# thalesfm/differentiable-renderer

Measured on AMD Instinct MI355X. Metric: Mray/s (fwd+bwd), Cornell 512x512 @64spp depth 8, higher is better.
Workload: dtype f32; 1 GPU; config 3: Cornell 512x512, 64 spp, depth 8, fwd + radiative backprop w.r.t. the albedos; scene 'cornell' (cornell box of render.cpp:26-59) 512x512, 64 spp per GPU, depth 8 (-b 8 -p 1), fwd + radiative-backprop gradients of 4 parameters; program=builtin, parallelism=1 GPU, gpu_max_hw_queues=4 (set by this script before the HIP runtime started)

## Files before the change

### differentiable-renderer_amd/csrc/drt_ctx.h

```cpp
#pragma once

namespace {

struct DevBuf {
    void* p = nullptr;
    size_t cap = 0;
};

struct TimedLaunch {
    int kernel;
    hipEvent_t e0, e1;
};

struct RenderJob {
    drt_camera_desc cam;
    drt_render_params rp;
    const float* adjoint_rgb = nullptr;
    float* out_rgb = nullptr;
    double* out_param_grad = nullptr;
    float* out_gimg = nullptr;
    drt_hip_stats* stats = nullptr;
    int gimg_param = -1;
    bool backward = false, dev_out = false, timing = false, want_segments = false, sync = true;
    bool zero_copy = false;
// ... 4 lines not shown
    uint32_t n_local_pixels = 0;
    size_t n_count_words = 0;
    float* d_out = nullptr;
    float* d_gimg = nullptr;
    size_t off_grad = 0, off_img = 0, off_gimg = 0, off_adj = 0, img_bytes = 0, grad_bytes = 0;
    drt_hip_stats st;
    std::chrono::steady_clock::time_point t0;
};

}

struct drt_hip_ctx {
    int device = 0;
    int n_cu = 256;
    uint64_t device_mem = (uint64_t)288 << 30;
    int mesh_blocks_per_cu = 4;
    hipStream_t stream = nullptr;
    std::string err;

    bool has_scene = false;
    bool has_specular = false;
    bool emissive_bxdf = false;
    int max_colour_param = -1;
    bool prog_ok = false;
    bool prog_sorted = false;
    unsigned long long prog_sig[4] = {0, 0, 0, 0};
    std::string arch = "gfx950";
    int jit_mode = 1;
    uint64_t scene_work = 0;
    std::map<std::string, hipFunction_t> jit_fn;
    std::vector<hipModule_t> jit_modules;
    std::string user_header;
    std::string jit_error;
    double jit_ms = 0;
    int n_params = 0, n_shapes = 0;
    int n_user_params = 0;
    int n_grad_slots = 0;
    std::vector<uint8_t> requires_grad;
    std::vector<drt_material_desc> materials;
    DevScene<float>* d_scene_f = nullptr;
    DevScene<double>* d_scene_d = nullptr;
    float* d_params_f = nullptr;
    double* d_params_d = nullptr;
    bool has_mesh = false;
    DevBvh<float> bvh_f{};
    DevBvh<double> bvh_d{};
// ... 114 lines not shown
```

### differentiable-renderer_amd/csrc/drt_path.h

```cpp
#pragma once

#include "drt_kernels.h"

#define DRT_DRAW_TABLE (3 * DRT_MAX_DEPTH + 8)

struct PathArgs {
    int32_t W, H, spp;
    int32_t shard, n_shards, band;
    uint32_t Pb, p0, Sb, s0, spr, n_ranges, n_groups;
    int32_t min_bounces, depth_cap, cap_is_roulette, cap_draws;
    uint32_t rr_threshold, seed, rng_stream;
    uint32_t regen_min;
    uint32_t shade_min, descend_min;
    int32_t gimg_param;
    uint32_t gen_rows, gen_clog2;
    uint32_t hist_lds, hist_stride;
    uint32_t gimg_row, pad_gen;
    unsigned long long hist_ovf;
    double p_rr, inv_p_rr;
    double eye[3], fwd[3], right[3], up[3];
    double tan_half, aspect, inv_W, inv_H;
    float p_rr_f, inv_p_rr_f;
    float eye_f[3], fwd_f[3], right_f[3], up_f[3], cs_step_f, ct_step_f;
};
// ... 70 lines not shown
            dst[i] = src[i];
    }
    {
        const int* src = reinterpret_cast<const int*>(sc->materials);
        int* dst = reinterpret_cast<int*>(lds.sc.materials);
        for (int i = threadIdx.x; i < nm * (int)(sizeof(DevMaterial<R>) / sizeof(int)); i += blockDim.x)
            dst[i] = src[i];
    }
    for (int i = threadIdx.x; i < ne; i += blockDim.x)
        lds.sc.emitter_param[i] = sc->emitter_param[i];
    for (int i = threadIdx.x; i < ns; i += blockDim.x)
        lds.sc.flat[i] = sc->flat[i];
#ifdef DRT_USER_SHAPES
    for (int i = threadIdx.x; i < ns * 4; i += blockDim.x)
        lds.user_q[i >> 2][i & 3] = sc->user_q[i >> 2][i & 3];
#endif
    const int np = sc->n_params < DRT_PATH_LDS_PARAMS ? sc->n_params : DRT_PATH_LDS_PARAMS;
    for (int i = threadIdx.x; i < np * 3; i += blockDim.x)
        lds.params[i] = params[i];
    __syncthreads();
}


template <typename R>
struct TangentLds {
    R colnz[DRT_FAST_PARAMS][4];
    R invc[DRT_FAST_PARAMS][4];
    uint32_t inc[DRT_FAST_PARAMS][4];
};

template <typename R, typename SL>
__device__ inline void stage_tangents(TangentLds<R>& tl, const SL& lds)
{
    if (threadIdx.x < DRT_FAST_PARAMS) {
        const int p = threadIdx.x;
        const bool in = p < lds.sc.n_params;
        uint32_t zinc = 0, zbits = 0;
#pragma unroll
        for (int ch = 0; ch < 3; ++ch) {
            const R c = in ? lds.params[p * 3 + ch] : R(1);
            const bool zero = abs_r(c) < R(1e-18);
            tl.colnz[p][ch] = zero ? R(1) : c;
            tl.invc[p][ch] = zero ? R(0) : R(1) / c;
            zinc |= zero ? 1u << (8 * ch) : 0u;
            zbits |= zero ? 1u << ch : 0u;
        }
        tl.colnz[p][3] = R(0);
        tl.invc[p][3] = R(0);
        tl.inc[p][0] = p < 4 ? 1u << (8 * p) : 0u;
        tl.inc[p][1] = p >= 4 ? 1u << (8 * (p - 4)) : 0u;
        tl.inc[p][2] = zinc;
        tl.inc[p][3] = zbits;
    }
    __syncthreads();
}

template <typename R, int NP, int NC>
struct Tangents {
    uint32_t cnt[NC > 4 ? 2 : 1];
    uint32_t zc;
    R* acc;
    __device__ inline V3<R> acc_get(int p) const { return mk<R>(acc[(p * 3) * DRT_BLOCK], acc[(p * 3 + 1) * DRT_BLOCK], acc[(p * 3 + 2) * DRT_BLOCK]); }
    __device__ inline void acc_set(int p, V3<R> v) { acc[(p * 3) * DRT_BLOCK] = v.x; acc[(p * 3 + 1) * DRT_BLOCK] = v.y; acc[(p * 3 + 2) * DRT_BLOCK] = v.z; }
    __device__ inline void new_path() { cnt[0] = 0; if (NC > 4) cnt[NC > 4 ? 1 : 0] = 0; zc = 0; }
};

#define DRT_NP_ANY (-1)
#ifndef DRT_LOCKSTEP_MIN_BLOCKS
#define DRT_LOCKSTEP_MIN_BLOCKS 7
#endif
#ifndef DRT_LOCKSTEP_GEN_MIN_BLOCKS
#define DRT_LOCKSTEP_GEN_MIN_BLOCKS 6
#endif
#ifndef DRT_LOCKSTEP_SPEC_MIN_BLOCKS
#define DRT_LOCKSTEP_SPEC_MIN_BLOCKS 6
// ... 143 lines not shown
    tg.gsum = mk<R>(R(0), R(0), R(0));
    tg.gimg_row = a.gimg_row;
    tg.hist_lds = a.hist_lds;
    tg.hist_stride = a.hist_stride;
    tg.clog2 = a.gen_clog2;
    tg.table = &gb.table[threadIdx.x / DRT_WAVE][threadIdx.x & ((1u << a.gen_clog2) - 1u)];
    tg.acc = nullptr;
    tg.new_path();
}
template <typename R>
__device__ inline void gen_finish(const GenBlock<R>& gb, const PathArgs& a, double* __restrict__ gpart)
{
    __syncthreads();
    const uint32_t copies = 1u << a.gen_clog2;
    for (uint32_t r = threadIdx.x; r < a.gen_rows; r += DRT_BLOCK) {
        double v = 0;
        for (int ww = 0; ww < DRT_BLOCK / DRT_WAVE; ++ww)
            for (uint32_t c = 0; c < copies; ++c)
                v += (double)gb.table[ww][(r << a.gen_clog2) + c];
        gpart[(size_t)blockIdx.x * a.gen_rows + r] = v;
    }
}

template <typename R, int NP, int NC, bool LOSS = false, typename SL = PathSceneLds<R>>
__device__ inline void add_emission(const SL& lds, const TangentLds<R>& tl, const R* __restrict__ params, uint32_t eid, R inv_pk,
                                    V3<R> T, V3<R> g, V3<R>& L, Tangents<R, NP, NC>& tg)
{
    const V3<R> E = load_param<R, (NP != 0)>(lds, params, (int)eid) * inv_pk;
    V3<R> Tr = T;
    if (NC > 0 || NP == DRT_NP_ANY)
        Tr = mk<R>((tg.zc & 0xFFu) ? R(0) : T.x, (tg.zc & 0xFF00u) ? R(0) : T.y, (tg.zc & 0xFF0000u) ? R(0) : T.z);
    L = L + Tr * E;
    if constexpr (NP == DRT_NP_ANY) {
        if (LOSS)
            g = mk<R>(R(2) * (L.x - g.x), R(2) * (L.y - g.y), R(2) * (L.z - g.z));
        const V3<R> gE = g * E;
        const uint32_t ebits = pid_unpack(tg.gl->invc[eid < DRT_PATH_LDS_PARAMS ? eid : 0][3]);
        if ((ebits & 0xFFFFu) != DRT_SLOT_NONE && eid < DRT_PATH_LDS_PARAMS)
            tg.add(ebits & 0xFFFFu, g * Tr * inv_pk);
        const V3<R> TgE = Tr * gE;
        const V3<R> U = mk<R>((tg.zc & 0xFFu) == 0x1u ? T.x * gE.x : R(0), (tg.zc & 0xFF00u) == 0x100u ? T.y * gE.y : R(0),
                              (tg.zc & 0xFF0000u) == 0x10000u ? T.z * gE.z : R(0));
        const uint32_t nw = tg.nv >> 2;
        for (uint32_t w = 0; wave_any(w < nw); ++w)
            tg.add_word(w < nw ? tg.load_word(w) : 0xFFFFFFFFu, TgE, U);
        tg.add_word(tg.cur, TgE, U);
    } else
    if constexpr (NP > 0) {
        if (NC > 0)
            asm volatile("" ::: "memory");
        if (LOSS)
            g = mk<R>(R(2) * (L.x - g.x), R(2) * (L.y - g.y), R(2) * (L.z - g.z));
        const V3<R> gE = g * E, gT = g * Tr * inv_pk;
#pragma unroll
        for (int p = 0; p < NP; ++p) {
            const bool own = eid == (uint32_t)p;
            const V3<R> ap = tg.acc_get(p);
            const V3<R> a0 = mk<R>(ap.x + (own ? gT.x : R(0)), ap.y + (own ? gT.y : R(0)), ap.z + (own ? gT.z : R(0)));
            if (p < NC) {
                const uint32_t n = (tg.cnt[p >> 2] >> (8 * (p & 3))) & 0xFFu;
                const R nf = (R)(int)n;
                V3<R> dT = mk<R>(Tr.x * (nf * tl.invc[p][0]), Tr.y * (nf * tl.invc[p][1]), Tr.z * (nf * tl.invc[p][2]));
                const uint32_t zb = __builtin_amdgcn_readfirstlane(tl.inc[p][3]);
                if (zb) {
                    const bool one = n == 1u;
                    if (zb & 1u) dT.x = (one && (tg.zc & 0xFFu) == 0x1u) ? T.x : R(0);
                    if (zb & 2u) dT.y = (one && (tg.zc & 0xFF00u) == 0x100u) ? T.y : R(0);
                    if (zb & 4u) dT.z = (one && (tg.zc & 0xFF0000u) == 0x10000u) ? T.z : R(0);
                }
                tg.acc_set(p, mk<R>(fma_r(dT.x, gE.x, a0.x), fma_r(dT.y, gE.y, a0.y), fma_r(dT.z, gE.z, a0.z)));
            } else
                tg.acc_set(p, a0);
        }
    }
}

template <typename R>
struct CameraLane {
    R cs0, ct0;
};

template <typename R>
struct PathVertex {
    V3<R> P, nrm, d;
    uint32_t ids;
    int material;
    bool hit, scattered;
};

template <typename R, bool SPEC, int NP, int NC, typename SG>
__device__ inline void path_bounce(const PathArgs& a, const PathSceneLds<R>& lds, const TangentLds<R>& tl, const DevScene<R>* __restrict__ sc,
                                   const R* __restrict__ params, const ProgRecs<SG::n, R>& recs, uint32_t key,
                                   R pk, R inv_pk, uint32_t n_theta, bool next_rr, bool next_cap, bool live, V3<R> g,
                                   typename Q4<R>::T& ra, typename Q2<R>::T& rb, V3<R>& T, V3<R>& L, Tangents<R, NP, NC>& tg,
                                   bool& alive, bool& capped, bool& on_light, uint32_t& light, PathVertex<R>* vo = nullptr,
                                   bool last = false, const float* __restrict__ seed_px = nullptr, const uint32_t* ih = nullptr)
{
    auto draw = [&](uint32_t n) { return ih ? drt_rng_combine(ih[n], key) : rng_draw(a.rng_stream, key, n); };
    const HitRec<R> h = path_closest_hit<SG>(sc, recs, ra, rb);
    const bool hit = live && h.prim >= 0;
    const int prim = h.prim >= 0 ? h.prim : 0;
    const V3<R> o = mk<R>(ra.x, ra.y, ra.z);
    const V3<R> d = mk<R>(ra.w, rb.x, rb.y);
    const V3<R> P = o + d * h.t;
    const DevShape<R>& sh = lds.sc.shapes[prim];
    const uint32_t ids = (uint32_t)sh.pad;
    const uint32_t cid = ids & 0xFFFFu, eid = ids >> 16;
    const bool has_bxdf = cid != DRT_ID_NONE, emits = hit && eid != DRT_ID_NONE;
    on_light = emits && !has_bxdf;
    light = eid;
    if (last && !vo) {
        if (wave_any(emits && has_bxdf)) {
            if (emits && has_bxdf) {
// ... 23 lines not shown
    if (vo) {
        vo->P = P; vo->nrm = nrm; vo->d = d;
        vo->ids = ids;
        vo->material = sh.material;
        vo->hit = hit;
        vo->scattered = hit && has_bxdf;
    }
    if (wave_any(emits && has_bxdf)) {
        if (emits && has_bxdf) {
            if (NP != 0 && seed_px)
                g = mk<R>((R)seed_px[0], (R)seed_px[1], (R)seed_px[2]);
            add_emission<R, NP, NC>(lds, tl, params, eid, inv_pk, T, g, L, tg);
        }
    }
    const DevMaterial<R>& m = lds.sc.materials[has_bxdf ? sh.material : 0];
    V3<R> wo;
    R q, bs;
    sample_bxdf<R, SPEC>(m, nrm, d, draw(n_theta), draw(n_theta + 1), wo, q, bs);
    const R c = dot(nrm, wo);
    const R mk_ = div_r(bs * c, q * pk);
    const bool rr_kills = next_rr && draw(n_theta + 2) < a.rr_threshold;
    alive = hit && has_bxdf && !next_cap && !rr_kills;
    capped = hit && has_bxdf && next_cap && !a.cap_is_roulette && !rr_kills;
    const int cidx = has_bxdf ? (int)cid : 0;
    V3<R> col;
    if constexpr (NP == DRT_NP_ANY) {
        const R* rec = tg.gl->colnz[cidx < DRT_PATH_LDS_PARAMS ? cidx : 0];
        col = mk<R>(rec[0], rec[1], rec[2]);
        tg.zc += alive ? pid_unpack(rec[3]) : 0u;
        if (ih)
            tg.template push<false>(alive, cid);
        else
            tg.template push<true>(live, alive ? cid : 0xFFu);
    } else
        col = NC > 0 ? mk<R>(tl.colnz[cidx][0], tl.colnz[cidx][1], tl.colnz[cidx][2]) : load_param<R, (NP > 0)>(lds, params, cidx);
    const V3<R> cmv = col * mk_;
    const V3<R> cm = mk<R>(alive ? cmv.x : R(1), alive ? cmv.y : R(1), alive ? cmv.z : R(1));
    if constexpr (NC > 0 && NP != DRT_NP_ANY) {
        tg.cnt[0] += alive ? tl.inc[cidx][0] : 0u;
        if (NC > 4)
            tg.cnt[NC > 4 ? 1 : 0] += alive ? tl.inc[cidx][1] : 0u;
        tg.zc += alive ? tl.inc[cidx][2] : 0u;
    }
    T = T * cm;
    const V3<R> no = P + wo * R(1e-3);
    ra.x = no.x; ra.y = no.y; ra.z = no.z; ra.w = wo.x;
    rb.x = wo.y; rb.y = wo.z;
}

#ifndef DRT_CAMERA_ARGS_F32
#define DRT_CAMERA_ARGS_F32 1
#endif
template <typename R, bool ARGS_F32 = (DRT_CAMERA_ARGS_F32 != 0)>
__device__ inline uint32_t path_camera(const PathArgs& a, const CameraLane<R>& cl, uint32_t gpix, uint32_t px, uint32_t py, uint32_t sl,
                                       typename Q4<R>::T& ra, typename Q2<R>::T& rb)
{
    const uint64_t path = (uint64_t)gpix * (uint64_t)a.spp + (uint64_t)(a.s0 + sl);
    const uint32_t key = (uint32_t)path;
    if (sizeof(R) == 4) {
        const float cs_step = ARGS_F32 ? a.cs_step_f : (float)(2. * a.aspect * a.tan_half * a.inv_W);
// ... 36 lines not shown
    return path_camera<R, false>(a, cl, gpix, px, py, sl, ra, rb);
}

#ifndef DRT_LEAN_MAX_SHAPES
#ifdef DRT_USER_SHAPES
#define DRT_LEAN_MAX_SHAPES (-1)
#else
#define DRT_LEAN_MAX_SHAPES 10
#endif
#endif
template <size_t RB, bool SPEC, int NP, int NSG, bool REGEN>
constexpr int path_min_blocks()
{
    if (RB == 4 && NP <= 4) {
        if (!REGEN)
            return SPEC ? ((NP == DRT_NP_ANY || NSG > DRT_LEAN_MAX_SHAPES) ? 5 : DRT_LOCKSTEP_SPEC_MIN_BLOCKS)
                        : (NP == DRT_NP_ANY ? DRT_LOCKSTEP_GEN_MIN_BLOCKS : (NSG <= DRT_LEAN_MAX_SHAPES ? DRT_LOCKSTEP_MIN_BLOCKS : DRT_LOCKSTEP_GEN_MIN_BLOCKS));
        return (NP == DRT_NP_ANY && NSG == 0) ? 4
                                              : (SPEC ? 5 : DRT_REGEN_MIN_BLOCKS);
    }
    return (RB == 8 && NP <= 4 && !REGEN && !SPEC) ? DRT_F64_MIN_BLOCKS : 1;
}

template <typename R, bool SPEC, int NP, int NC, typename SG, bool REGEN = false, bool LOSS = false>
__global__ void __launch_bounds__(DRT_BLOCK, (path_min_blocks<sizeof(R), SPEC, NP, SG::n, REGEN>()))
k_path(PathArgs a, const DevScene<R>* __restrict__ sc, const R* __restrict__ params, const float* __restrict__ adjoint,
       double* __restrict__ gpart, double* __restrict__ fpart, uint32_t* __restrict__ counts,
       unsigned long long* __restrict__ total, double* __restrict__ gimg_part)
{
    if (total && blockIdx.x == 0 && threadIdx.x < 8)
        total[threadIdx.x] = 0;
    typedef typename Q4<R>::T R4;
    typedef typename Q2<R>::T R2;
    __shared__ PathSceneLds<R> lds;
    __shared__ double s_red[REGEN ? 1 : DRT_BLOCK / DRT_WAVE][DRT_FAST_PARAMS * 3];
    __shared__ TangentLds<R> s_tl;
    constexpr bool GEN = NP == DRT_NP_ANY;
    __shared__ typename PickT<GEN, GenBlock<R>, NoLds>::T s_gen;
    extern __shared__ uint32_t s_hist[];
    if constexpr (GEN)
        gen_zero(s_gen);
    stage_path_scene(lds, sc, params);
    const TangentLds<R>& tl = s_tl;
    if (NC > 0 && !GEN)
        stage_tangents(s_tl, lds);

    const uint32_t lane = threadIdx.x & (DRT_WAVE - 1);
    const uint32_t w = grid_wave();
    const uint32_t range = w / a.n_groups, group = w - range * a.n_groups;
    const uint32_t lp = group * DRT_WAVE + lane;
    const bool have = range < a.n_ranges && lp < a.Pb;
    const uint32_t s_begin = range * a.spr;
    const uint32_t s_end = s_begin + a.spr < a.Sb ? s_begin + a.spr : a.Sb;

    Tangents<R, NP, NC> tg;
    __shared__ R s_acc[NP > 0 ? NP * 3 : 1][DRT_BLOCK];
// ... 41 lines not shown
    if (range < a.n_ranges && !REGEN) {
    for (uint32_t sl = s_begin; sl < s_end; ++sl) {
        R4 ra;
        R2 rb;
        const uint32_t key = path_camera<R, ARGS_F32>(a, cl, gpix, px, py, sl, ra, rb);
        bool live = have && a.depth_cap > 0 && !(a.min_bounces <= 0 && rng_draw(a.rng_stream, key, 2) < a.rr_threshold);
        V3<R> T = mk<R>(R(1), R(1), R(1)), L = mk<R>(R(0), R(0), R(0));
        uint32_t end_ids = DRT_ID_NONE;
        R end_inv_pk = R(1);
        if (NC > 0 || GEN)
            tg.new_path();
        for (int kk = 0; kk < a.depth_cap; ++kk) {
            const uint32_t n_live = (uint32_t)__popcll(wave_ballot(live));
            if (n_live == 0)
                break;
            n_seg += n_live;
            const R pk = kk >= a.min_bounces ? pk_rr : R(1);
            const R inv_pk = kk >= a.min_bounces ? inv_p_rr : R(1);
            const uint32_t n_theta = draw_offset(kk, 0, a.min_bounces) + camera_draw_base(a.min_bounces);
            const bool next_rr = (kk + 1) >= a.min_bounces;
            const bool next_cap = (kk + 1) >= a.depth_cap;
            bool alive, capped, on_light;
            uint32_t light;
            path_bounce<R, SPEC, NP, NC, SG>(a, lds, tl, sc, params, recs, key, pk, inv_pk, n_theta, next_rr, next_cap, live, g,
                                                    ra, rb, T, L, tg, alive, capped, on_light, light, nullptr, next_cap);
            end_ids = on_light ? light : end_ids;
            end_inv_pk = on_light ? inv_pk : end_inv_pk;
            if (next_cap && !a.cap_is_roulette)
                n_capped += (uint32_t)__popcll(wave_ballot(capped));
            live = alive;
        }
        if (wave_any(end_ids != DRT_ID_NONE)) {
            if (end_ids != DRT_ID_NONE)
                add_emission<R, NP, NC, LOSS>(lds, tl, params, end_ids, end_inv_pk, T, g, L, tg);
        }
        fx += (double)L.x; fy += (double)L.y; fz += (double)L.z;
    }
    }
    __shared__ R s_pcs[REGEN ? DRT_BLOCK : 1], s_pct[REGEN ? DRT_BLOCK : 1];
    __shared__ uint32_t s_pgpix[REGEN ? DRT_BLOCK : 1];
    __shared__ double s_film[REGEN ? 3 : 1][REGEN ? DRT_BLOCK : 1];
    __shared__ uint32_t s_ih[REGEN ? DRT_DRAW_TABLE : 1];
    if (REGEN) {
        for (uint32_t n = threadIdx.x; n < DRT_DRAW_TABLE; n += DRT_BLOCK)
            s_ih[REGEN ? n : 0] = drt_rng_index_hash(a.rng_stream, n);
        s_pcs[threadIdx.x] = cl.cs0;
        s_pct[threadIdx.x] = cl.ct0;
        s_pgpix[threadIdx.x] = have ? gpix : 0xFFFFFFFFu;
        s_film[0][threadIdx.x] = 0.0; s_film[REGEN ? 1 : 0][threadIdx.x] = 0.0; s_film[REGEN ? 2 : 0][threadIdx.x] = 0.0;
        __syncthreads();
    }
    if (range < a.n_ranges && REGEN) {
        const uint32_t wbase = threadIdx.x & ~(uint32_t)(DRT_WAVE - 1);
        const uint32_t n_items = DRT_WAVE * (s_end - s_begin);
        uint32_t n_next = 0;
        uint32_t key = 0, pix = wbase, pgpix = 0;
        int kk = 0;
// ... 452 lines not shown
```

### differentiable-renderer_amd/csrc/drt_render_impl.h

```cpp
#pragma once

namespace {

int timing_begin(drt_hip_ctx* ctx, bool on, int kernel)
{
    if (!on)
        return DRT_OK;
    while (ctx->event_pool.size() < ctx->events_used + 2) {
        hipEvent_t e;
        HIPCHK(ctx, hipEventCreate(&e));
        ctx->event_pool.push_back(e);
    }
    TimedLaunch t;
    t.kernel = kernel;
    t.e0 = ctx->event_pool[ctx->events_used++];
    t.e1 = ctx->event_pool[ctx->events_used++];
    HIPCHK(ctx, hipEventRecord(t.e0, ctx->stream));
    ctx->timed.push_back(t);
    return DRT_OK;
}

int timing_end(drt_hip_ctx* ctx, bool on)
{
    if (!on)
// ... 92 lines not shown
    return b ? f(std::true_type()) : f(std::false_type());
}
template <int V, int... Vs, typename F>
auto with_int(int v, F&& f)
{
    if constexpr (sizeof...(Vs) == 0)
        return v == V ? f(IntC<V>()) : decltype(f(IntC<V>()))();
    else
        return v == V ? f(IntC<V>()) : with_int<Vs...>(v, f);
}
inline int np_width(int n_params, int general)
{
    return n_params <= 4 ? 4 : (n_params <= 8 ? 8 : general);
}

enum class PathOp { biased, unbiased, mesh };
enum class PathProg { cornell, sorted, scene };
struct PathForm {
    PathOp op;
    bool f64, spec;
    int np, nc;
    bool regen;
    bool loss;
    PathProg prog;
};

template <typename R>
struct Shard {
    typedef typename Q4<R>::T R4;
    typedef typename Q2<R>::T R2;
    drt_hip_ctx* ctx;
    const drt_camera_desc* cam;
    const drt_render_params* rp;
    const float* d_adjoint;
    float* d_out_rgb;
    bool backward, timing;
    drt_hip_stats* st;
    uint32_t n_local_pixels;
    int D;
    double* film;
    int gimg_param;
    double* gfilm;
    float* d_out_gimg;
    const DevScene<R>* d_scene;
    const R* d_params;
    DevBvh<R> bvh;
// ... 56 lines not shown
        if (forced > 0)
            return forced < left ? forced : left;
        double alive = 1.0;
        int n = 0;
        while (n < left && n < 8) {
            alive *= 0.93 * ((k + n + 1) >= rp->min_bounces && (k + n + 1) < D ? 1.0 - rp->absorb : 1.0);
            ++n;
            if (alive < 0.1)
                break;
        }
        return n;
    }
};

inline std::string path_kernel_name(const drt_hip_ctx* ctx, const PathForm& f)
{
    const std::string sg = drt_jit::sig_type(ctx->prog_sig, ctx->n_shapes);
    const char* type = f.f64 ? "double" : "float";
    const char* sp = f.spec ? "true" : "false";
    char name[400];
    if (f.op == PathOp::unbiased)
        snprintf(name, sizeof name, "k_path_unbiased<%s, %s, %d, %s>", type, sp, f.np, sg.c_str());
    else
        snprintf(name, sizeof name, "k_path<%s, %s, %d, %d, %s, %s%s>", type, sp, f.np, f.nc, sg.c_str(), f.regen ? "true" : "false", f.loss ? ", true" : "");
    return name;
}

template <typename R>
const void* library_path_kernel(const PathForm& f)
{
    if (f.loss || f.prog == PathProg::scene)
        return nullptr;
    const auto columns = [&f](auto k) {
        if (f.np == DRT_NP_ANY && f.nc == 0) return k(IntC<DRT_NP_ANY>(), IntC<0>());
        if (f.np == 8 && f.nc == 8) return k(IntC<8>(), IntC<8>());
        if (f.np == 4 && f.nc == 3) return k(IntC<4>(), IntC<3>());
        if (f.np == 4 && f.nc == 4) return k(IntC<4>(), IntC<4>());
        if (f.np == 0 && f.nc == 0) return k(IntC<0>(), IntC<0>());
        return (const void*)nullptr;
    };
    const auto spec_sig = [&f](auto k) {
        return with_bool(f.spec, [&](auto spec) { return with_bool(f.prog == PathProg::cornell, [&](auto cornell) {
            return k(spec, std::conditional_t<cornell, SigCornell, SigNone>()); }); });
    };
    if (f.op == PathOp::mesh)
        return columns([&f](auto np, auto nc) {
            return with_bool(f.spec, [](auto spec) { return (const void*)k_path_mesh<R, spec, decltype(np)::value, decltype(nc)::value>; });
        });
    if (f.op == PathOp::unbiased)
        return with_int<DRT_NP_ANY, 8, 4>(f.np, [&](auto np) {
            return spec_sig([](auto spec, auto sg) { return (const void*)k_path_unbiased<R, spec, decltype(np)::value, decltype(sg)>; });
        });
    if (f.nc == 1)
        return f.np != DRT_NP_ANY || f.regen ? nullptr
                                             : spec_sig([](auto spec, auto sg) { return (const void*)k_path<R, spec, DRT_NP_ANY, 1, decltype(sg), false>; });
    return columns([&](auto np, auto nc) {
        return spec_sig([&](auto spec, auto sg) {
            return with_bool(f.regen, [](auto regen) {
                return (const void*)k_path<R, decltype(spec)::value, decltype(np)::value, decltype(nc)::value, decltype(sg), regen>;
            });
        });
    });
}

template <typename R>
void shard_plan(Shard<R>& s)
{
// ... 16 lines not shown
    PathForm& f = s.path;
    const bool lane_is_pixel = s.gimg_param >= 0 && !s.mesh_path;
    f.regen = (tuning().path_regen > 0 || s.mesh_path) && !s.unbiased && !lane_is_pixel;
    if (s.use_path && !s.mesh_path && !lane_is_pixel && tuning().path_regen < 0 && !s.unbiased) {
        double alive = 1.0, mean_len = 0.0;
        int longest = D;
        for (int k = 0; k < D; ++k) {
            mean_len += alive;
            alive *= 0.975 * ((k + 1) >= rp->min_bounces ? 1.0 - rp->absorb : 1.0);
            if (alive < 1.0 / 256 && longest == D)
                longest = k + 1;
        }
        f.regen = 1.7 * mean_len + 0.5 < (double)longest;
    }
    const bool gen = tangents && ctx->n_params <= DRT_PATH_LDS_PARAMS &&
                     (s.gimg_param >= 0 ? ctx->n_params > DRT_FAST_PARAMS && !s.mesh_path
                                        : ctx->n_params > tuning().gen_above && (tuning().path_general || ctx->n_params <= DRT_FAST_PARAMS));
    f.op = s.unbiased ? PathOp::unbiased : (s.mesh_path ? PathOp::mesh : PathOp::biased);
    f.f64 = sizeof(R) == 8; f.spec = ctx->has_specular;
    f.np = !tangents ? 0 : (gen ? DRT_NP_ANY : np_width(ctx->n_params, DRT_NP_ANY));
    f.nc = !tangents ? 0 : gen ? (s.gimg_param >= 0 ? 1 : 0)
                             : (f.np == 8 ? 8 : (ctx->max_colour_param < 3 ? 3 : 4));
    f.loss = s.loss_l2;
    if (s.use_path && s.loss_l2) {
        s.use_path = false;
        if ((sizeof(R) == 4 || !ctx->user_header.empty()) && !ctx->emissive_bxdf && ctx->jit_mode >= DRT_SPECIALISE_AUTO) {
            s.loss_kernel = jit_function(ctx, path_kernel_name(ctx, f), ctx->jit_mode > DRT_SPECIALISE_AUTO || !ctx->user_header.empty());
            s.use_path = s.loss_kernel != nullptr;
        }
    }
    s.path_gen = s.use_path && gen;
    const bool builtin = tuning().builtin_program && ctx->jit_mode >= 0 && ctx->n_shapes == DRT_NSIG_CORNELL &&
                         ctx->prog_sig[0] == DRT_SIG_CORNELL && !s.loss_kernel && !s.mesh_path &&
                         ctx->user_header.empty();
    f.prog = builtin ? PathProg::cornell : ((s.loss_kernel || !ctx->user_header.empty()) ? PathProg::scene : PathProg::sorted);
    uint64_t cap_default;
    {
        const uint64_t f = sizeof(R) / 4;
        const uint64_t per_path = f * (112u + 8u * (uint64_t)(D > 0 ? D : 1) + (ctx->has_mesh ? 36u : 0u) + (s.unbiased ? (ctx->has_mesh ? 186u : 110u) : 0u)) + 24u;
        const uint64_t budget = std::min<uint64_t>(ctx->device_mem / 8, (uint64_t)32 << 30);
        cap_default = (uint64_t)1 << 22;
        while (cap_default < ((uint64_t)1 << 28) && 2 * cap_default * per_path <= budget)
            cap_default *= 2;
        if (!s.use_path && rp->batch_paths <= 0 && (uint64_t)ctx->ray_a[0].cap < std::min<uint64_t>(cap_default, s.total_paths) * 16u * f) {
            size_t free_b = 0, total_b = 0;
            if (hipMemGetInfo(&free_b, &total_b) == hipSuccess)
// ... 253 lines not shown
        if (d_adjoint) {
            HIPCHK(ctx, hipEventRecord(ctx->ev_begin[lane2], ctx->stream));
            HIPCHK(ctx, hipStreamWaitEvent(ks, ctx->ev_begin[lane2], 0));
        }
        if (ctx->lane_used[lane2] && ctx->ev_lane_free[lane2])
            HIPCHK(ctx, hipStreamWaitEvent(ks, ctx->ev_lane_free[lane2], 0));
        if (ctx->params_pending[lane2] && ctx->ev_params) {
            HIPCHK(ctx, hipStreamWaitEvent(ks, ctx->ev_params, 0));
            ctx->params_pending[lane2] = false;
        }
    }
    PathForm form = s.path;
    hipFunction_t jit = s.loss_kernel;
    ctx->scene_work += (uint64_t)a.n_paths * (uint64_t)(s.D > 0 ? s.D : 1);
    if (form.prog == PathProg::sorted && form.op != PathOp::mesh && ctx->jit_mode > 0 && !form.f64 &&
        (ctx->jit_mode > 1 || ctx->scene_work >= DRT_JIT_AFTER_WORK) && (jit = jit_function(ctx, path_kernel_name(ctx, form), ctx->jit_mode > 1)))
        form.prog = PathProg::scene;
    if (form.prog == PathProg::scene && !jit) {
        jit = jit_function(ctx, path_kernel_name(ctx, form), true);
        if (!jit)
            return fail(ctx, DRT_ERR_UNSUPPORTED, ("render: the scene's caller-defined shape kinds did not compile: " + ctx->jit_error).c_str());
    }
    const void* fn = library_path_kernel<R>(form);
    if (!jit && !fn)
        return fail(ctx, DRT_ERR_UNSUPPORTED, "render: the library carries no path kernel of this form");
    st->path_program = form.prog == PathProg::cornell ? DRT_PROGRAM_BUILTIN : (jit ? DRT_PROGRAM_SPECIALISED : DRT_PROGRAM_SORTED);
    int rc;
    if ((rc = timing_begin(ctx, s.timing, DRT_K_PATH)) != DRT_OK) return rc;
    uint32_t* ovf = s.mesh_path ? (uint32_t*)ctx->mesh_ovf[(s.overlap_ok && lane2) ? 1 : 0].p : (uint32_t*)nullptr;
    uint32_t ovf_stride = (uint32_t)gpath * DRT_BLOCK;
    pa.hist_stride = ovf_stride;
    if (gen && hist_ovf_words > 0) {
        DevBuf& hb = s.mesh_path ? ctx->mesh_ovf[(s.overlap_ok && lane2) ? 1 : 0] : ctx->hist_ovf[(s.overlap_ok && lane2) ? 1 : 0];
        const size_t words = (size_t)hist_ovf_words + (s.mesh_path ? (size_t)(DRT_BVH_STACK - DRT_MESH_LDS_STACK) : 0);
        int rce;
        if ((rce = ensure(ctx, hb, words * ovf_stride * sizeof(uint32_t))) != DRT_OK) return rce;
        if (s.mesh_path) {
            ovf = (uint32_t*)hb.p;
            pa.hist_ovf = (unsigned long long)(uintptr_t)(ovf + (size_t)(DRT_BVH_STACK - DRT_MESH_LDS_STACK) * ovf_stride);
        } else
            pa.hist_ovf = (unsigned long long)(uintptr_t)hb.p;
    }
    pa.gimg_row = DRT_SLOT_NONE;
    if (gen && s.gimg_param >= 0 && s.gimg_param < DRT_PATH_LDS_PARAMS && ctx->requires_grad[(size_t)s.gimg_param]) {
        uint32_t row = 0;
        for (int p2 = 0; p2 < s.gimg_param; ++p2)
// ... 363 lines not shown
```

### differentiable-renderer_amd/csrc/drt_scene.h

```cpp
#pragma once

namespace {

template <typename R4>
int upload_array(drt_hip_ctx* ctx, const std::vector<R4>& host, const R4** dev)
{
    void* p = nullptr;
    hipError_t e = hipMalloc(&p, host.empty() ? 16 : host.size() * sizeof(R4));
    if (e == hipSuccess && !host.empty())
        e = hipMemcpy(p, host.data(), host.size() * sizeof(R4), hipMemcpyHostToDevice);
    if (e != hipSuccess) {
        ctx->err = std::string("mesh upload: ") + hipGetErrorString(e);
        if (p) (void)hipFree(p);
        return DRT_ERR_HIP;
    }
    ctx->mesh_allocs.push_back(p);
    *dev = (const R4*)p;
    return DRT_OK;
}

inline float link_bits(float, uint32_t v) { float f; memcpy(&f, &v, 4); return f; }
inline double link_bits(double, uint32_t v) { return (double)v; }

template <typename R>
// ... 287 lines not shown
        return DRT_OK;
    };
    if (rc == DRT_OK) rc = up((void**)&ctx->d_scene_f, hf, sizeof *hf);
    if (rc == DRT_OK) rc = up((void**)&ctx->d_scene_d, hd, sizeof *hd);
    if (rc == DRT_OK) rc = up((void**)&ctx->d_params_f, pf.data(), pf.size() * sizeof(float));
    if (rc == DRT_OK) rc = up((void**)&ctx->d_params_d, pd.data(), pd.size() * sizeof(double));
    const int n_dev_params = hf->n_params;
    ctx->n_grad_slots = hf->n_grad_slots;
    ctx->prog_ok = hf->prog_ok != 0;
    ctx->prog_sorted = hf->prog_sorted != 0;
    if (memcmp(ctx->prog_sig, sig, sizeof ctx->prog_sig) != 0 || ctx->n_shapes != s->n_shapes || ctx->user_header != user_header) {
        for (int i = 0; i < 2; ++i)
            if (ctx->path_stream[i])
                (void)hipStreamSynchronize(ctx->path_stream[i]);
        for (hipModule_t m : ctx->jit_modules)
            (void)hipModuleUnload(m);
        ctx->jit_modules.clear();
        ctx->jit_fn.clear();
    }
    for (int i = 0; i < 4; ++i)
        ctx->prog_sig[i] = sig[i];
    ctx->user_header = user_header;
    ctx->max_colour_param = -1;
    for (int i = 0; i < hf->n_materials; ++i)
        ctx->max_colour_param = std::max(ctx->max_colour_param, hf->materials[i].param);
    delete hf;
    delete hd;
    if (rc != DRT_OK)
        return rc;
    release_mesh(ctx);
    {
        std::vector<drt_bvh::Tri> tris;
        int max_face_param = -1;
        uint32_t flat = 0;
        double lo[3] = {INFINITY, INFINITY, INFINITY}, hi[3] = {-INFINITY, -INFINITY, -INFINITY};
        for (int i = 0; i < s->n_shapes; ++i) {
            const drt_shape_desc& sh = s->shapes[i];
            if (sh.type != DRT_SHAPE_MESH) { ++flat; continue; }
            const drt_mesh_desc& m = s->meshes[sh.mesh];
            for (int k = 0; k < m.n_triangles; ++k, ++flat) {
                drt_bvh::Tri t;
                const double* a = &m.vertices[(size_t)m.indices[k * 3] * 3];
                const double* b = &m.vertices[(size_t)m.indices[k * 3 + 1] * 3];
                const double* c = &m.vertices[(size_t)m.indices[k * 3 + 2] * 3];
                for (int x = 0; x < 3; ++x) {
                    t.v0[x] = a[x]; t.e1[x] = b[x] - a[x]; t.e2[x] = c[x] - a[x];
                    lo[x] = std::min(lo[x], std::min(a[x], std::min(b[x], c[x])));
                    hi[x] = std::max(hi[x], std::max(a[x], std::max(b[x], c[x])));
// ... 125 lines not shown
```

### differentiable-renderer_amd/csrc/drt_tuning.h

```cpp
#pragma once

#include <cstdlib>
#include <cstring>

namespace {

struct Tuning {
    int jit = 1;
    bool jit_verbose = false;
    bool builtin_program = true;
    bool overlap_frames = true;
    int path_spr = 0;
    int path_regen = -1;
    int path_regen_min = 8;
    bool path_general = true;
    int gen_above = 4;
    int gen_hist_lds = -1;
    int gen_copies_log2 = -1;
    long long batch_paths = 0;
    int region_size = 0;
    int shade_bounces = 0;
    int mesh_blocks_per_cu = 0;
    int tail_bounces = 0;
    int shade_list_group = 4;
    int bvh_refill = -1;
    int bvh_descend_min = -1;
    long long mesh_path_max = 1 << 20;
    int mesh_shade_min = 32;
    int copy_blocks = 64;
    bool sync_zero_copy = true;
    int sync_spin_us = 2000;
    bool async_copy_inline = false;
    bool group_threads = true;
    long long dump_path = -1;
};

inline const Tuning& tuning()
{
    static const Tuning t = [] {
        Tuning v;
        auto num = [](const char* name, long long dflt) { const char* e = getenv(name); return e ? atoll(e) : dflt; };
        auto off = [](const char* name) { const char* e = getenv(name); return e && atoi(e) == 0; };
        if (const char* e = getenv("DRT_HIP_JIT"))
            v.jit = !strcmp(e, "force") ? 2 : (atoi(e) > 0 ? 1 : (atoi(e) < 0 ? -1 : 0));
        v.jit_verbose = getenv("DRT_HIP_JIT_VERBOSE") != nullptr;
        v.builtin_program = !off("DRT_HIP_BUILTIN_PROGRAM");
        v.overlap_frames = !off("DRT_HIP_OVERLAP_FRAMES");
        v.path_spr = (int)num("DRT_HIP_PATH_SPR", 0);
        v.path_regen = (int)num("DRT_HIP_PATH_REGEN", -1);
        v.path_regen_min = (int)num("DRT_HIP_PATH_REGEN_MIN", 8);
        v.path_general = !off("DRT_HIP_PATH_GENERAL");
        v.gen_copies_log2 = (int)num("DRT_HIP_GEN_COPIES_LOG2", -1);
        v.gen_above = (int)num("DRT_HIP_GEN_ABOVE", 4);
        if (v.gen_above < 0) v.gen_above = 0;
        if (v.gen_above > DRT_FAST_PARAMS) v.gen_above = DRT_FAST_PARAMS;
        v.gen_hist_lds = (int)num("DRT_HIP_GEN_HIST_LDS", -1);
        if (v.gen_hist_lds > 16) v.gen_hist_lds = 16;
        if (v.gen_copies_log2 > 4) v.gen_copies_log2 = 4;
        v.batch_paths = num("DRT_HIP_BATCH_PATHS", 0);
        v.region_size = (int)num("DRT_HIP_REGION_SIZE", 0);
        v.shade_bounces = (int)num("DRT_HIP_SHADE_BOUNCES", 0);
        v.mesh_blocks_per_cu = (int)num("DRT_HIP_MESH_BLOCKS_PER_CU", 0);
        v.shade_list_group = (int)num("DRT_HIP_SHADE_LIST_GROUP", 4);
        v.tail_bounces = (int)num("DRT_HIP_TAIL_BOUNCES", 0);
        if (v.tail_bounces < 0 || v.tail_bounces > 2) v.tail_bounces = 0;
        v.bvh_refill = (int)num("DRT_HIP_BVH_REFILL", -1);
        v.bvh_descend_min = (int)num("DRT_HIP_BVH_DESCEND_MIN", -1);
        v.mesh_path_max = num("DRT_HIP_MESH_PATH_MAX", 1 << 20);
        v.mesh_shade_min = (int)num("DRT_HIP_MESH_SHADE_MIN", 32);
        v.copy_blocks = (int)num("DRT_HIP_COPY_BLOCKS", 64);
        v.sync_zero_copy = !off("DRT_HIP_SYNC_ZERO_COPY");
// ... 23 lines not shown
```

Measured before the change: 195,400 Mray/s.

## Specialise path kernel on per-parameter colour/emission roles and branchless tangent counters

Records at scene load which fast parameters are material colours and which are emitters, and encodes these role masks into the k_path template argument. add_emission can then skip parameters with no role and resolve ownership at compile time when a single parameter is the emitter. A Cornell-specific f32 instantiation is added, with a fallback to the generic kernel when none matches. Separately, path_bounce gains a freeze-by-row mode that adds a neutral 'rest' row to the tangent LDS tables, so dead paths index a unit colour and zero increment instead of going through selects. This adds another kernel instantiation and more template complexity, and the role masks must match the scene or gradients will be wrong.

After: 201,700 Mray/s (median of 6 runs). 1.03x the previous value.

```diff
diff --git a/differentiable-renderer_amd/csrc/drt_ctx.h b/differentiable-renderer_amd/csrc/drt_ctx.h
--- a/differentiable-renderer_amd/csrc/drt_ctx.h
+++ b/differentiable-renderer_amd/csrc/drt_ctx.h
@@ -50,6 +50,7 @@
     bool has_specular = false;
     bool emissive_bxdf = false;
     int max_colour_param = -1;
+    unsigned colour_mask = 0, emission_mask = 0;
     bool prog_ok = false;
     bool prog_sorted = false;
     unsigned long long prog_sig[4] = {0, 0, 0, 0};
diff --git a/differentiable-renderer_amd/csrc/drt_path.h b/differentiable-renderer_amd/csrc/drt_path.h
--- a/differentiable-renderer_amd/csrc/drt_path.h
+++ b/differentiable-renderer_amd/csrc/drt_path.h
@@ -116,11 +116,15 @@
 }
 
 
+#define DRT_TANGENT_REST DRT_FAST_PARAMS
+#ifndef DRT_FREEZE_BY_ROW
+#define DRT_FREEZE_BY_ROW 1
+#endif
 template <typename R>
 struct TangentLds {
-    R colnz[DRT_FAST_PARAMS][4];
+    R colnz[DRT_FAST_PARAMS + (DRT_FREEZE_BY_ROW != 0)][4];
     R invc[DRT_FAST_PARAMS][4];
-    uint32_t inc[DRT_FAST_PARAMS][4];
+    uint32_t inc[DRT_FAST_PARAMS + (DRT_FREEZE_BY_ROW != 0)][4];
 };
 
 template <typename R, typename SL>
@@ -145,6 +149,10 @@
         tl.inc[p][1] = p >= 4 ? 1u << (8 * (p - 4)) : 0u;
         tl.inc[p][2] = zinc;
         tl.inc[p][3] = zbits;
+    }
+    if (DRT_FREEZE_BY_ROW != 0 && threadIdx.x >= DRT_WAVE && threadIdx.x < DRT_WAVE + 4) {
+        tl.colnz[DRT_TANGENT_REST][threadIdx.x - DRT_WAVE] = R(1);
+        tl.inc[DRT_TANGENT_REST][threadIdx.x - DRT_WAVE] = 0u;
     }
     __syncthreads();
 }
@@ -334,7 +342,21 @@
     }
 }
 
-template <typename R, int NP, int NC, bool LOSS = false, typename SL = PathSceneLds<R>>
+#define DRT_NC_ROLES(nc, colour_mask, emission_mask) ((int)(nc) | (int)(colour_mask) << 8 | (int)(emission_mask) << 16)
+#define DRT_NC_OF(ncr) ((int)(ncr) & 0xFF)
+#define DRT_ROLES_OF(ncr) ((int)(ncr) >> 8)
+#define DRT_ROLES_CORNELL DRT_ROLES_OF(DRT_NC_ROLES(0, 0x7, 0x8))
+template <int NP, int NC, int ROLES>
+struct PathRoles {
+    static constexpr int all = NP > 0 ? (1 << NP) - 1 : 0;
+    static constexpr int colm = ROLES ? (ROLES & 0xFF) & ((1 << NC) - 1) : (1 << NC) - 1;
+    static constexpr int emitm = ROLES ? (ROLES >> 8) & all : all;
+    static __device__ constexpr bool colour(int p) { return (colm >> p) & 1; }
+    static __device__ constexpr bool emission(int p) { return (emitm >> p) & 1; }
+    static __device__ constexpr bool only_emission(int p) { return emitm == (1 << p); }
+};
+
+template <typename R, int NP, int NC, bool LOSS = false, typename SL = PathSceneLds<R>, int ROLES = 0>
 __device__ inline void add_emission(const SL& lds, const TangentLds<R>& tl, const R* __restrict__ params, uint32_t eid, R inv_pk,
                                     V3<R> T, V3<R> g, V3<R>& L, Tangents<R, NP, NC>& tg)
 {
@@ -366,10 +388,16 @@
         const V3<R> gE = g * E, gT = g * Tr * inv_pk;
 #pragma unroll
         for (int p = 0; p < NP; ++p) {
-            const bool own = eid == (uint32_t)p;
+            typedef PathRoles<NP, NC, ROLES> RL;
+            const bool is_colour = (RL::colm >> p) & 1, is_emission = (RL::emitm >> p) & 1;
+            if (ROLES != 0 && !is_colour && !is_emission)
+                continue;
+            const bool own = (ROLES != 0 && RL::emitm == (1 << p)) || eid == (uint32_t)p;
             const V3<R> ap = tg.acc_get(p);
-            const V3<R> a0 = mk<R>(ap.x + (own ? gT.x : R(0)), ap.y + (own ? gT.y : R(0)), ap.z + (own ? gT.z : R(0)));
-            if (p < NC) {
+            V3<R> a0 = mk<R>(ap.x + (own ? gT.x : R(0)), ap.y + (own ? gT.y : R(0)), ap.z + (own ? gT.z : R(0)));
+            if (ROLES != 0 && !is_emission)
+                a0 = ap;
+            if (is_colour) {
                 const uint32_t n = (tg.cnt[p >> 2] >> (8 * (p & 3))) & 0xFFu;
                 const R nf = (R)(int)n;
                 V3<R> dT = mk<R>(Tr.x * (nf * tl.invc[p][0]), Tr.y * (nf * tl.invc[p][1]), Tr.z * (nf * tl.invc[p][2]));
@@ -400,7 +428,7 @@
     bool hit, scattered;
 };
 
-template <typename R, bool SPEC, int NP, int NC, typename SG>
+template <typename R, bool SPEC, int NP, int NC, typename SG, bool FREEZE_BY_ROW = false>
 __device__ inline void path_bounce(const PathArgs& a, const PathSceneLds<R>& lds, const TangentLds<R>& tl, const DevScene<R>* __restrict__ sc,
                                    const R* __restrict__ params, const ProgRecs<SG::n, R>& recs, uint32_t key,
                                    R pk, R inv_pk, uint32_t n_theta, bool next_rr, bool next_cap, bool live, V3<R> g,
@@ -470,7 +498,8 @@
     const bool rr_kills = next_rr && draw(n_theta + 2) < a.rr_threshold;
     alive = hit && has_bxdf && !next_cap && !rr_kills;
     capped = hit && has_bxdf && next_cap && !a.cap_is_roulette && !rr_kills;
-    const int cidx = has_bxdf ? (int)cid : 0;
+    constexpr bool REST = FREEZE_BY_ROW && NC > 0 && NP != DRT_NP_ANY;
+    const int cidx = REST ? (alive ? (int)cid : DRT_TANGENT_REST) : (has_bxdf ? (int)cid : 0);
     V3<R> col;
     if constexpr (NP == DRT_NP_ANY) {
         const R* rec = tg.gl->colnz[cidx < DRT_PATH_LDS_PARAMS ? cidx : 0];
@@ -482,8 +511,14 @@
             tg.template push<true>(live, alive ? cid : 0xFFu);
     } else
         col = NC > 0 ? mk<R>(tl.colnz[cidx][0], tl.colnz[cidx][1], tl.colnz[cidx][2]) : load_param<R, (NP > 0)>(lds, params, cidx);
-    const V3<R> cmv = col * mk_;
-    const V3<R> cm = mk<R>(alive ? cmv.x : R(1), alive ? cmv.y : R(1), alive ? cmv.z : R(1));
+    const V3<R> cmv = col * (REST ? (alive ? mk_ : R(1)) : mk_);
+    const V3<R> cm = REST ? cmv : mk<R>(alive ? cmv.x : R(1), alive ? cmv.y : R(1), alive ? cmv.z : R(1));
+    if constexpr (REST) {
+        tg.cnt[0] += tl.inc[cidx][0];
+        if (NC > 4)
+            tg.cnt[NC > 4 ? 1 : 0] += tl.inc[cidx][1];
+        tg.zc += tl.inc[cidx][2];
+    } else
     if constexpr (NC > 0 && NP != DRT_NP_ANY) {
         tg.cnt[0] += alive ? tl.inc[cidx][0] : 0u;
         if (NC > 4)
@@ -566,7 +601,7 @@
     return (RB == 8 && NP <= 4 && !REGEN && !SPEC) ? DRT_F64_MIN_BLOCKS : 1;
 }
 
-template <typename R, bool SPEC, int NP, int NC, typename SG, bool REGEN = false, bool LOSS = false>
+template <typename R, bool SPEC, int NP, int NCR, typename SG, bool REGEN = false, bool LOSS = false>
 __global__ void __launch_bounds__(DRT_BLOCK, (path_min_blocks<sizeof(R), SPEC, NP, SG::n, REGEN>()))
 k_path(PathArgs a, const DevScene<R>* __restrict__ sc, const R* __restrict__ params, const float* __restrict__ adjoint,
        double* __restrict__ gpart, double* __restrict__ fpart, uint32_t* __restrict__ counts,
@@ -576,6 +611,7 @@
         total[threadIdx.x] = 0;
     typedef typename Q4<R>::T R4;
     typedef typename Q2<R>::T R2;
+    constexpr int NC = DRT_NC_OF(NCR), ROLES = DRT_ROLES_OF(NCR);
     __shared__ PathSceneLds<R> lds;
     __shared__ double s_red[REGEN ? 1 : DRT_BLOCK / DRT_WAVE][DRT_FAST_PARAMS * 3];
     __shared__ TangentLds<R> s_tl;
@@ -663,7 +699,7 @@
             const bool next_cap = (kk + 1) >= a.depth_cap;
             bool alive, capped, on_light;
             uint32_t light;
-            path_bounce<R, SPEC, NP, NC, SG>(a, lds, tl, sc, params, recs, key, pk, inv_pk, n_theta, next_rr, next_cap, live, g,
+            path_bounce<R, SPEC, NP, NC, SG, (DRT_FREEZE_BY_ROW != 0 && sizeof(R) == 4 && !SPEC && SG::n <= DRT_LEAN_MAX_SHAPES)>(a, lds, tl, sc, params, recs, key, pk, inv_pk, n_theta, next_rr, next_cap, live, g,
                                                     ra, rb, T, L, tg, alive, capped, on_light, light, nullptr, next_cap);
             end_ids = on_light ? light : end_ids;
             end_inv_pk = on_light ? inv_pk : end_inv_pk;
@@ -673,7 +709,7 @@
         }
         if (wave_any(end_ids != DRT_ID_NONE)) {
             if (end_ids != DRT_ID_NONE)
-                add_emission<R, NP, NC, LOSS>(lds, tl, params, end_ids, end_inv_pk, T, g, L, tg);
+                add_emission<R, NP, NC, LOSS, PathSceneLds<R>, ROLES>(lds, tl, params, end_ids, end_inv_pk, T, g, L, tg);
         }
         fx += (double)L.x; fy += (double)L.y; fz += (double)L.z;
     }
diff --git a/differentiable-renderer_amd/csrc/drt_render_impl.h b/differentiable-renderer_amd/csrc/drt_render_impl.h
--- a/differentiable-renderer_amd/csrc/drt_render_impl.h
+++ b/differentiable-renderer_amd/csrc/drt_render_impl.h
@@ -138,6 +138,7 @@
     int np, nc;
     bool regen;
     bool loss;
+    int roles;
     PathProg prog;
 };
 
@@ -240,7 +241,7 @@
     if (f.op == PathOp::unbiased)
         snprintf(name, sizeof name, "k_path_unbiased<%s, %s, %d, %s>", type, sp, f.np, sg.c_str());
     else
-        snprintf(name, sizeof name, "k_path<%s, %s, %d, %d, %s, %s%s>", type, sp, f.np, f.nc, sg.c_str(), f.regen ? "true" : "false", f.loss ? ", true" : "");
+        snprintf(name, sizeof name, "k_path<%s, %s, %d, %d, %s, %s%s>", type, sp, f.np, DRT_NC_ROLES(f.nc, 0, 0) | f.roles << 8, sg.c_str(), f.regen ? "true" : "false", f.loss ? ", true" : "");
     return name;
 }
 
@@ -261,6 +262,14 @@
         return with_bool(f.spec, [&](auto spec) { return with_bool(f.prog == PathProg::cornell, [&](auto cornell) {
             return k(spec, std::conditional_t<cornell, SigCornell, SigNone>()); }); });
     };
+    if (f.roles != 0) {
+        if constexpr (sizeof(R) == 4) {
+            if (f.op == PathOp::biased && !f.spec && !f.regen && f.np == 4 && f.nc == 3 && f.roles == DRT_ROLES_CORNELL)
+                return with_bool(f.prog == PathProg::cornell, [](auto cornell) {
+                    return (const void*)k_path<R, false, 4, DRT_NC_ROLES(3, 0, 0) | DRT_ROLES_CORNELL << 8, std::conditional_t<cornell, SigCornell, SigNone>, false>; });
+        }
+        return nullptr;
+    }
     if (f.op == PathOp::mesh)
         return columns([&f](auto np, auto nc) {
             return with_bool(f.spec, [](auto spec) { return (const void*)k_path_mesh<R, spec, decltype(np)::value, decltype(nc)::value>; });
@@ -323,6 +332,10 @@
     f.nc = !tangents ? 0 : gen ? (s.gimg_param >= 0 ? 1 : 0)
                              : (f.np == 8 ? 8 : (ctx->max_colour_param < 3 ? 3 : 4));
     f.loss = s.loss_l2;
+    f.roles = 0;
+    if (tuning().path_roles && tangents && !gen && sizeof(R) == 4 && !f.spec && !f.regen && !f.loss && f.op == PathOp::biased && s.gimg_param < 0 &&
+        ctx->colour_mask != 0 && ctx->emission_mask != 0)
+        f.roles = (int)(ctx->colour_mask | ctx->emission_mask << 8);
     if (s.use_path && s.loss_l2) {
         s.use_path = false;
         if ((sizeof(R) == 4 || !ctx->user_header.empty()) && !ctx->emissive_bxdf && ctx->jit_mode >= DRT_SPECIALISE_AUTO) {
@@ -622,6 +635,10 @@
             return fail(ctx, DRT_ERR_UNSUPPORTED, ("render: the scene's caller-defined shape kinds did not compile: " + ctx->jit_error).c_str());
     }
     const void* fn = library_path_kernel<R>(form);
+    if (!jit && !fn && form.roles != 0) {
+        form.roles = 0;
+        fn = library_path_kernel<R>(form);
+    }
     if (!jit && !fn)
         return fail(ctx, DRT_ERR_UNSUPPORTED, "render: the library carries no path kernel of this form");
     st->path_program = form.prog == PathProg::cornell ? DRT_PROGRAM_BUILTIN : (jit ? DRT_PROGRAM_SPECIALISED : DRT_PROGRAM_SORTED);
diff --git a/differentiable-renderer_amd/csrc/drt_scene.h b/differentiable-renderer_amd/csrc/drt_scene.h
--- a/differentiable-renderer_amd/csrc/drt_scene.h
+++ b/differentiable-renderer_amd/csrc/drt_scene.h
@@ -333,8 +333,15 @@
         ctx->prog_sig[i] = sig[i];
     ctx->user_header = user_header;
     ctx->max_colour_param = -1;
-    for (int i = 0; i < hf->n_materials; ++i)
+    ctx->colour_mask = ctx->emission_mask = 0;
+    for (int i = 0; i < hf->n_materials; ++i) {
         ctx->max_colour_param = std::max(ctx->max_colour_param, hf->materials[i].param);
+        if (hf->materials[i].param >= 0 && hf->materials[i].param < DRT_FAST_PARAMS)
+            ctx->colour_mask |= 1u << hf->materials[i].param;
+    }
+    for (int i = 0; i < hf->n_emitters; ++i)
+        if (hf->emitter_param[i] >= 0 && hf->emitter_param[i] < DRT_FAST_PARAMS)
+            ctx->emission_mask |= 1u << hf->emitter_param[i];
     delete hf;
     delete hd;
     if (rc != DRT_OK)
diff --git a/differentiable-renderer_amd/csrc/drt_tuning.h b/differentiable-renderer_amd/csrc/drt_tuning.h
--- a/differentiable-renderer_amd/csrc/drt_tuning.h
+++ b/differentiable-renderer_amd/csrc/drt_tuning.h
@@ -11,6 +11,7 @@
     bool builtin_program = true;
     bool overlap_frames = true;
     int path_spr = 0;
+    bool path_roles = true;
     int path_regen = -1;
     int path_regen_min = 8;
     bool path_general = true;
@@ -47,6 +48,7 @@
         v.builtin_program = !off("DRT_HIP_BUILTIN_PROGRAM");
         v.overlap_frames = !off("DRT_HIP_OVERLAP_FRAMES");
         v.path_spr = (int)num("DRT_HIP_PATH_SPR", 0);
+        v.path_roles = !off("DRT_HIP_PATH_ROLES");
         v.path_regen = (int)num("DRT_HIP_PATH_REGEN", -1);
         v.path_regen_min = (int)num("DRT_HIP_PATH_REGEN_MIN", 8);
         v.path_general = !off("DRT_HIP_PATH_GENERAL");
```
